# lowmee/xchu_slam

Hardware: AMD Instinct MI355X
Metric: NDT scans/sec (120k-pt scan vs 200k-voxel localmap, 30 iters) at 1/2/4/8 GPUs; % HBM BW (higher is better)
Workload: dtype f32 (f64 accumulate)

## Files before the change

### xchu_slam_amd/csrc/host_sort.hip

```cpp
#include "ndt_host.h"

namespace ndt::host {

ndt_status scan_ctx(ndt_ctx* c, Lane L, int nb, ScanCtx* sc) {
    sc->tickets = c->opt.tile_tickets ? 1 : 0;
    if ((size_t)nb > L.s.scan_status.cap) {
        TRY(ensure(c, L.s.scan_status, (size_t)nb));
        HIPCHK(c, hipMemsetAsync(L.s.scan_status.p, 0, L.s.scan_status.cap * sizeof(unsigned long long), L.st));
    }
    if (!L.s.scan_ticket.p) {
        TRY(ensure(c, L.s.scan_ticket, 1));
        HIPCHK(c, hipMemsetAsync(L.s.scan_ticket.p, 0, sizeof(unsigned long long), L.st));
        L.s.scan_tickets = 0;
    }
    sc->status = L.s.scan_status.p;
    sc->ticket = L.s.scan_ticket.p;
    sc->ticket_base = L.s.scan_tickets;
    sc->epoch = ++L.s.scan_epoch;
    sc->nb = nb;
    if (sc->tickets) L.s.scan_tickets += (unsigned long long)nb;
    return NDT_OK;
}

ndt_status enqueue_scan(ndt_ctx* c, Lane L, const int* in, int n_host, const int* n_dev, int* out, int* total_out, GridHeader* herr) {
    const int nb = std::max(1, ceil_div(n_host, kTileKeys));
    ScanCtx sc;
    TRY(scan_ctx(c, L, nb, &sc));
    hipLaunchKernelGGL(k_scan_onepass, dim3(nb), dim3(kBlock), 0, L.st, in, n_host, n_dev, out, total_out, sc, herr);
    return NDT_OK;
}

constexpr int kRadixWideKeys = 4 << 20;
int radix_items(const ndt_ctx* c, int n) {
    return ceil_div(n, kTileKeys) < c->n_cu ? 4 : (n >= kRadixWideKeys ? 24 : 16);
}
size_t radix_status_words(int nb) { return (size_t)4 * 256 * ((size_t)nb + (size_t)ceil_div(nb, 16)); }
void launch_radix_pass(const ndt_ctx* c, Lane L, int items, int nb, int* k0, int* v0, int* k1, int* v1, int n, int pass,
                       const GridHeader* h, GridHeader* herr, int last_pass) {
    auto* kern = items == 4 ? k_radix_onesweep<4> : items == 16 ? k_radix_onesweep<16> : k_radix_onesweep<24>;
    hipLaunchKernelGGL(kern, dim3(nb), dim3(kBlock), 0, L.st, k0, v0, k1, v1, n, pass, h, L.s.radix_aux.p, L.s.radix_status.p, nb,
                       herr, last_pass, c->opt.tile_tickets ? 1 : 0);
}

int radix_launch_passes(const ndt_ctx* c) {
    if (c->rerun_full) return 4;
    return c->opt.radix_force > 0 ? std::min(c->opt.radix_force, 4) : c->radix_pred;
}
void note_grid_width(ndt_ctx* c, long long cells, int dense) {
    if (cells <= 0) return;
    const long long top = dense ? cells - 1 : cells;
    int bits = 0;
    while (bits < 31 && (top >> bits) != 0) ++bits;
    c->radix_pred = std::min(4, std::max(1, (bits + 1 + 7) / 8));
}

ndt_status enqueue_bin_and_sort(ndt_ctx* c, Lane L, const float4* pts, int n, int dense, GridHeader* h, float leaf, int layout,
                                int binning, int2* cloud_span, int passes) {
    if (&L.s == &c->s && !cloud_span) c->inc_ok = false;
    const int nb_mm = std::max(1, std::min(ceil_div(n, 4 * kBlock), 1024));
    TRY(ensure(c, L.s.mm, (size_t)nb_mm * 7));
    const int items = radix_items(c, n);
    const int nb_sort = std::max(1, ceil_div(n, kBlock * items));
    const size_t n_kv = cloud_span ? (size_t)n + (size_t)n / 4 : (size_t)n;
    TRY(ensure(c, L.s.k0, n_kv)); TRY(ensure(c, L.s.v0, n_kv)); TRY(ensure(c, L.s.k1, n_kv)); TRY(ensure(c, L.s.v1, n_kv));
    TRY(ensure(c, L.s.radix_aux, kRadixAuxWords));
    TRY(ensure(c, L.s.radix_status, radix_status_words(nb_sort)));
    TRY(ensure(c, L.s.seg_start, (size_t)n + 1));
    hipLaunchKernelGGL(k_minmax, dim3(nb_mm), dim3(kBlock), 0, L.st, pts, n, dense, L.s.mm.p, L.s.radix_aux.p,
                       cloud_span ? c->d_clk.p + 3 : nullptr, nullptr, nullptr, nullptr);
    const int nb_keys = std::max(1, std::min(ceil_div(n, 4 * kBlock), 512));
    hipLaunchKernelGGL(k_keys, dim3(nb_keys), dim3(kBlock), 0, L.st, pts, n, dense, L.s.mm.p, nb_mm, h, leaf, c->prm.min_points_per_voxel,
                       c->prm.min_covar_eigvalue_mult, layout, binning, L.s.k0.p, L.s.v0.p, L.s.radix_aux.p, L.s.radix_status.p,
                       (int)radix_status_words(nb_sort), cloud_span ? c->grid.p : nullptr, (long long)c->grid.cap, cloud_span ? c->table.p : nullptr,
                       1LL << c->max_log2cap, nullptr, 0);
    for (int pass = 0; pass < passes; ++pass)
        launch_radix_pass(c, L, items, nb_sort, L.s.k0.p, L.s.v0.p, L.s.k1.p, L.s.v1.p, n, pass, h, h, passes - 1);
    const int nb_seg = std::max(1, ceil_div(n, kTileKeys));
    ScanCtx sc;
    TRY(scan_ctx(c, L, nb_seg, &sc));
    hipLaunchKernelGGL(k_seg_scan, dim3(nb_seg), dim3(kBlock), 0, L.st, L.s.k0.p, L.s.k1.p, n, h, L.s.seg_start.p, sc);
    if (cloud_span) {
        ScanCtx sc2;
        TRY(scan_ctx(c, L, nb_seg, &sc2));
        hipLaunchKernelGGL(k_cloud_scan, dim3(nb_seg), dim3(kBlock), 0, L.st, L.s.seg_start.p, n, h, cloud_span, sc2, c->max_log2cap);
    }
    return NDT_OK;
}

ndt_status enqueue_downsample_finalize(ndt_ctx* c, Lane L, const GridHeader* h, const float4* in, int n, float4* out) {
    TRY(ensure(c, L.s.sorted_pts, std::max(n, 1)));
    const int nb = std::max(1, std::min(ceil_div(n, 4 * kBlock), 2048));
    hipLaunchKernelGGL(k_sorted_gather, dim3(nb), dim3(kBlock), 0, L.st, in, L.s.v0.p, L.s.v1.p, h, L.s.sorted_pts.p, n);
    hipLaunchKernelGGL(k_downsample_finalize, dim3(std::max(1, ceil_div(n, kBlock))), dim3(kBlock), 0, L.st, L.s.sorted_pts.p,
                       L.s.seg_start.p, h, out);
    HIPCHK(c, hipGetLastError());
    return NDT_OK;
}

}
```

### xchu_slam_amd/csrc/host_target.hip

```cpp
#include "ndt_host.h"

namespace ndt::host {

namespace {

ndt_status grow_grid(ndt_ctx* c) {
    const long long want_cells = std::min<long long>(std::max<long long>(2 * c->grid_cells_seen, 16ll << 20), 1ll << 30);
    if ((long long)c->grid.cap < want_cells) TRY(ensure(c, c->grid, (size_t)want_cells));
    return NDT_OK;
}

ndt_status alloc_cloud_buffers(ndt_ctx* c, size_t max_cloud) {
    TRY(ensure(c, c->recs, max_cloud)); TRY(ensure(c, c->cent, max_cloud)); TRY(ensure(c, c->icovd, max_cloud * 9));
    TRY(ensure(c, c->evals, max_cloud * 3)); TRY(ensure(c, c->cloud_key, max_cloud));
    return NDT_OK;
}

constexpr int kFinalize3WavesMaxPoints = 4 << 20;

ndt_status prepare_target_buffers(ndt_ctx* c, int M, int* nb_cloud) {
    TRY(grow_grid(c));
    const size_t max_cloud = std::max(1, M / std::max(1, c->prm.min_points_per_voxel) + 1);
    TRY(alloc_cloud_buffers(c, max_cloud));
    unsigned l = 6;
    while (l < 30 && (1ull << l) < 4ull * max_cloud) ++l;
    c->max_log2cap = l;
    TRY(ensure(c, c->table, (size_t)1 << l));
    *nb_cloud = std::max(1, ceil_div((long long)max_cloud, kBlock));
    TRY(ensure(c, c->s.cloud_span, (size_t)*nb_cloud * kBlock));
    TRY(ensure(c, c->valid_part, max_cloud / 64 + 1));
    return NDT_OK;
}

ndt_status launch_finalize(ndt_ctx* c, int M, int nb_cloud) {
    auto* fin = M < kFinalize3WavesMaxPoints ? k_leaf_finalize<3> : k_leaf_finalize<2>;
    hipLaunchKernelGGL(fin, dim3(nb_cloud), dim3(kBlock), 0, c->stream.get(), c->target_ptr, c->s.k0.p, c->s.k1.p, c->s.v0.p,
                       c->s.v1.p, c->s.cloud_span.p, c->d_hdr.p, c->recs.p, c->cent.p, c->icovd.p, c->cloud_key.p,
                       c->evals.p, c->grid.p, c->table.p, c->valid_part.p);
    HIPCHK(c, hipGetLastError());
    return NDT_OK;
}

ndt_status enqueue_target_build(ndt_ctx* c) {
    c->inc_ok = false;
    ++c->n_builds_full;
    const int M = c->M;
    int nb_cloud = 0;
    TRY(prepare_target_buffers(c, M, &nb_cloud));
    TRY(enqueue_bin_and_sort(c, main_lane(c), c->target_ptr, M, c->target_dense, c->d_hdr.p, c->prm.resolution, 0, c->prm.precision_mode == 2 ? 1 : 0,
                             c->s.cloud_span.p, radix_launch_passes(c)));
    TRY(launch_finalize(c, M, nb_cloud));
    c->inc_ok = c->prm.precision_mode != 2 && c->target_dense == 1 && M > 0;
    return NDT_OK;
}

ndt_status enqueue_target_append(ndt_ctx* c, int n_old, int n_new, const float4* new_src) {
    const int M = n_old + n_new;
    int nb_cloud = 0;
    TRY(prepare_target_buffers(c, M, &nb_cloud));
    Lane Q{c->stream.get(), c->s_inc};
    float4* copy_to = new_src ? const_cast<float4*>(c->target_ptr) + n_old : nullptr;
    const float4* pts_new = new_src ? new_src : c->target_ptr + n_old;
    const int nq = std::max(n_new, 1);
    const int nb_mm = std::max(1, std::min(ceil_div(nq, 4 * kBlock), 1024));
    TRY(ensure(c, Q.s.mm, (size_t)nb_mm * 7));
    const int items = radix_items(c, nq);
    const int nb_sort = std::max(1, ceil_div(nq, kBlock * items));
    TRY(ensure(c, Q.s.k0, nq)); TRY(ensure(c, Q.s.v0, nq)); TRY(ensure(c, Q.s.k1, nq)); TRY(ensure(c, Q.s.v1, nq));
    TRY(ensure(c, Q.s.radix_aux, kRadixAuxWords));
    TRY(ensure(c, Q.s.radix_status, radix_status_words(nb_sort)));
    TRY(ensure(c, c->s.seg_start, (size_t)M + 1));
    hipLaunchKernelGGL(k_minmax, dim3(nb_mm), dim3(kBlock), 0, c->stream.get(), pts_new, n_new, 1, Q.s.mm.p, Q.s.radix_aux.p, c->d_clk.p + 3,
                       c->d_hdr.p, c->d_hdr_prev.p, copy_to);
    if (c->tgt_ev_valid) HIPCHK(c, hipEventRecord(c->ev_tgt.get(), c->stream.get()));
    const long long clear_words = std::max<long long>((long long)c->grid.cap, 2LL << c->max_log2cap) / 4;
    const int nb_keys = std::max(1, (int)std::min<long long>(std::max<long long>(ceil_div(nq, 4 * kBlock), ceil_div(clear_words, 4LL * kBlock)), 512));
    hipLaunchKernelGGL(k_keys, dim3(nb_keys), dim3(kBlock), 0, c->stream.get(), pts_new, n_new, 1, Q.s.mm.p, nb_mm, c->d_hdr.p, c->prm.resolution,
                       c->prm.min_points_per_voxel, c->prm.min_covar_eigvalue_mult, 0, 0, Q.s.k0.p, Q.s.v0.p, Q.s.radix_aux.p,
                       Q.s.radix_status.p, (int)radix_status_words(nb_sort), c->grid.p, (long long)c->grid.cap, c->table.p, 1LL << c->max_log2cap,
                       c->d_hdr_prev.p, n_old);
    const int passes = radix_launch_passes(c);
    for (int pass = 0; pass < passes; ++pass)
        launch_radix_pass(c, Q, items, nb_sort, Q.s.k0.p, Q.s.v0.p, Q.s.k1.p, Q.s.v1.p, n_new, pass, c->d_hdr.p, c->d_hdr.p, passes - 1);
    hipLaunchKernelGGL(k_merge_append, dim3(std::max(1, ceil_div(M, kMergeTileKeys))), dim3(kBlock), 0, c->stream.get(), c->s.k0.p, c->s.v0.p,
                       c->s.k1.p, c->s.v1.p, c->d_hdr_prev.p, n_old, Q.s.k0.p, Q.s.v0.p, Q.s.k1.p, Q.s.v1.p, n_new, c->d_hdr.p,
                       c->target_ptr);
    const Lane L = main_lane(c);
    const int nb_seg = std::max(1, ceil_div(M, kTileKeys));
    ScanCtx sc, sc2;
    TRY(scan_ctx(c, L, nb_seg, &sc));
    hipLaunchKernelGGL(k_seg_scan, dim3(nb_seg), dim3(kBlock), 0, c->stream.get(), c->s.k0.p, c->s.k1.p, M, c->d_hdr.p, c->s.seg_start.p, sc);
    TRY(scan_ctx(c, L, nb_seg, &sc2));
    hipLaunchKernelGGL(k_cloud_scan, dim3(nb_seg), dim3(kBlock), 0, c->stream.get(), c->s.seg_start.p, M, c->d_hdr.p, c->s.cloud_span.p, sc2,
                       c->max_log2cap);
    TRY(launch_finalize(c, M, nb_cloud));
    return NDT_OK;
}

}

ndt_status build_target(ndt_ctx* c) {
    ++c->tgt_gen;
    c->tgt_ev_valid = c->lanes.fit_tgt_used;
    if (c->tgt_ev_valid) HIPCHK(c, hipEventRecord(c->ev_tgt.get(), c->stream.get()));
    TRY(enqueue_target_build(c));
    c->build_unchecked = true;
    c->built_since_align = true;
    c->grid_valid = true;
    c->fit_valid = false;
    c->grid_res = c->prm.resolution;
    c->have_result = false;
    return NDT_OK;
}

ndt_status rerun_build(ndt_ctx* c, int berr) {
    ++c->n_builds_rerun;
    if (berr & kBuildErrLookback) {
        c->opt.tile_tickets = true;
        ++c->n_rerun_lookback;
    }
    c->inc_ok = false;
    c->rerun_full = true;
    const ndt_status st = build_target(c);
    c->rerun_full = false;
    return st;
}

ndt_status settle_build(ndt_ctx* c) {
    if (!c->build_unchecked || !c->grid_valid) return NDT_OK;
    for (int attempt = 0;; ++attempt) {
        HIPCHK(c, hipMemcpyAsync(c->h_hdr.get(), c->d_hdr.p, sizeof(GridHeader), hipMemcpyDeviceToHost, c->stream.get()));
        HIPCHK(c, hipStreamSynchronize(c->stream.get()));
        const int berr = c->h_hdr->pad[0];
        if (!berr) break;
        if (attempt > 0) return fail(c, NDT_EDEVICE, "target build failed twice (error bits " + std::to_string(berr) + ")");
        TRY(rerun_build(c, berr));
    }
    c->build_unchecked = false;
    note_grid_width(c, c->h_hdr->cells, c->target_dense);
    return NDT_OK;
}

ndt_status upload_points(ndt_ctx* c, DevBuf<float4>& dst, const float* xyz, size_t n, size_t stride_bytes) {
    TRY(ensure(c, dst, n));
    std::vector<float4> tmp(n);
    const char* base = reinterpret_cast<const char*>(xyz);
    for (size_t i = 0; i < n; ++i) {
        const float* f = reinterpret_cast<const float*>(base + i * stride_bytes);
        tmp[i] = make_float4(f[0], f[1], f[2], 1.0f);
    }
    if (n) HIPCHK(c, hipMemcpyAsync(dst.p, tmp.data(), n * sizeof(float4), hipMemcpyHostToDevice, c->stream.get()));
    HIPCHK(c, hipStreamSynchronize(c->stream.get()));
    return NDT_OK;
}

static ndt_status append_target(ndt_ctx* c, const float4* d_new, const float* h_new, size_t n, size_t stride_bytes) {
    TRY(set_dev(c));
    TRY(main_after_fit(c, false));
    if (n == 0) return NDT_OK;
    const size_t m0 = c->has_target ? (size_t)c->M : 0, m = m0 + n;
    if (m > 0x7fffffffULL) return fail(c, NDT_EINVAL, "target too large");
// ... 151 lines not shown
```

### xchu_slam_amd/csrc/ndt_kernels.h

```cpp
#pragma once
#include <hip/hip_runtime.h>
#include "ndt_types.h"
#include "ndt_linalg.h"
#include "ndt_icp.h"
#include "ndt_sc.h"
#include "ndt_isc.h"
#include "ndt_pgo.h"
#include "ndt_map.h"

namespace ndt {
__global__ void k_minmax(const float4*, int, int, float*, int*, unsigned long long*, const GridHeader*, GridHeader*, float4*);
__global__ void k_keys(const float4*, int, int, const float*, int, GridHeader*, float, int, double, int, int, int*, int*, int*, unsigned*, int,
                       int*, long long, int2*, long long, const GridHeader*, int);
__global__ void k_merge_append(int*, int*, int*, int*, const GridHeader*, int, const int*, const int*, const int*, const int*, int,
                               GridHeader*, const float4*);
template <int ITEMS>
__global__ void k_radix_onesweep(int*, int*, int*, int*, int, int, const GridHeader*, int*, unsigned*, int, GridHeader*, int, int);
__global__ void k_scan_onepass(const int*, int, const int*, int*, int*, ScanCtx, GridHeader*);
__global__ void k_seg_scan(const int*, const int*, int, GridHeader*, int*, ScanCtx);
__global__ void k_cloud_scan(const int*, int, GridHeader*, int2*, ScanCtx, unsigned);

template <int WAVES>
__global__ void k_leaf_finalize(const float4*, const int*, const int*, const int*, const int*, const int2*, GridHeader*,
                                VoxelRec*, float4*, double*, int*, double*, int*, int2*, int*);
__global__ void k_sorted_gather(const float4*, const int*, const int*, const GridHeader*, float4*, int);
__global__ void k_src_keys(const float4*, int, Mat4f, const GridHeader*, int*, int*, int*, unsigned*, int);
__global__ void k_src_gather(const float4*, const int*, const int*, const GridHeader*, float4*, int);
__global__ void k_crop_flags(const float4*, int, double, double, int*);
__global__ void k_compact4(const float4*, const int*, const int*, int, float4*);
template <int C>
__global__ void k_sor_knn(const float4*, int, int, const GridHeader*, const int*, const int*, const float4*, float*);
__global__ void k_sor_stats(const float*, int, double, double*);
__global__ void k_sor_keep(const float*, int, const double*, int*);
__global__ void k_ror_keep(const float4*, int, double, int, const GridHeader*, const int*, const int*, const float4*, int*);
__global__ void k_downsample_finalize(const float4*, const int*, const GridHeader*, float4*);
__global__ void k_fit_gather(const float4*, const int*, const int*, const int*, const int*, const int*, int, const GridHeader*, float4*,
                             int*, int*, int*);
__global__ void k_icp_pass(float4*, int, IcpState*, const GridHeader*, const int*, const int*, const float4*, const int*, int*, float*,
                           double*, unsigned*, IcpRecordDev*);
__global__ void k_sc_make(const float4*, int, unsigned*);
__global__ void k_sc_finalize(const unsigned*, ScDb, int);
__global__ void k_sc_detect(ScDb, const int*, const int*, int, int, ScDetectArgs, ndt_sc_result*);
__global__ void k_isc_make(const float4*, int, IscGeom, unsigned*);
__global__ void k_isc_finalize(const unsigned*, IscDb, int, int, int, double, double, double, double);
__global__ void k_isc_detect(IscDb, const int*, int, IscDetectArgs, IscPartial*);
__global__ void k_isc_reduce(const IscPartial*, const int*, int, int, IscDetectArgs, ndt_isc_result*);
__global__ void k_pgo_optimize(PgoGraph, PgoArgs);
__global__ void k_map_stack(const float4*, const int*, const long long*, const Mat4f*, int, int, int, float4*);
__global__ void k_fit_block_flags(const int*, const GridHeader*, int*);
__global__ void k_append2(const float4*, const float4*, int, const GridHeader*, float4*, float4*);
__global__ void k_fit_block_clear(int*, const GridHeader*);
__global__ void k_fit_tables(const int*, const int*, const int*, const int*, const GridHeader*, int*, int*);
__global__ void k_fitness(const float4*, int, Mat4f, const GridHeader*, const int*, const int*, const float4*, double, float*, double*,
                          int*, unsigned*, double*, long long*);
__global__ void k_score_radius(const float4*, int, Mat4f, const GridHeader*, const int2*, const int*, const VoxelRec*, const float4*,
                               const double*, double, double, double, float, double*);
template <int SEARCH, int PPT, bool ONE_TILE>
__global__ void k_pass_direct(const float4*, int, int, const GridHeader*, const int2*, const int*, const VoxelRec*, const AlignState*,
                              AlignState*, double*, unsigned*, double*, PassRecordDev*, int, int, unsigned long long*, int4*);
__global__ void k_pass_radius(const float4*, int, const GridHeader*, const int2*, const int*, const VoxelRec*, const float4*,
                              const double*, const AlignState*, AlignState*, double*, unsigned*, double*, PassRecordDev*, int, int,
                              unsigned long long*);
__global__ void k_transform(const float4*, int, const AlignState*, float4*);
__global__ void k_transform_mat(const float4*, int, Mat4f, float4*);
__global__ void k_align_init(const AlignState, AlignState*, unsigned*, unsigned long long*, int, unsigned long long*, const GridHeader*,
                             unsigned long long, const uint4*, uint4*, long long);
__global__ void k_copy16(const uint4*, uint4*, size_t);
__global__ void k_readback(const unsigned long long*, unsigned long long*, int, const unsigned long long*, unsigned long long*, int,
                           const unsigned long long*, unsigned long long*, int, const unsigned long long*, unsigned long long*,
                           unsigned long long*, unsigned long long, unsigned long long*, const GridHeader*);
hipError_t dbg_read_blk(unsigned long long* host, size_t count);
__global__ void k_svd_resume(AlignState*);
template <int SEARCH, bool ONE_TILE>
__global__ void k_pass_lead(const float4*, int, int, const GridHeader*, const int2*, const int*, const VoxelRec*, const AlignState*,
                            AlignState*, const double*, double*, PassRecordDev*, int, unsigned long long*, int4*);
}
```

### xchu_slam_amd/csrc/ndt_types.h

```cpp
#pragma once
#include <stdint.h>

namespace ndt {

constexpr int kBlock = 256;
constexpr int kLeadBlock = 512;
constexpr int kLeadBlock1 = 768;
#ifndef NDT_SPLIT_ACC
#define NDT_SPLIT_ACC 1
#endif
#ifndef NDT_LEAD_ONE_TILE
#define NDT_LEAD_ONE_TILE NDT_SPLIT_ACC
#endif
#ifndef NDT_DIRECT_ONE_TILE
#define NDT_DIRECT_ONE_TILE 0
#endif
constexpr int kDirectBlock = 256;
#ifndef NDT_PACKED_PAIR
#define NDT_PACKED_PAIR 1
#endif
#ifndef NDT_ROW_TRIPLE
#define NDT_ROW_TRIPLE 1
#endif
#ifndef NDT_NBR_CACHE
#define NDT_NBR_CACHE 1
#endif
__host__ __device__ constexpr int pass_block(int search, bool lead, bool one_tile = false) {
    return search == 1  ? kBlock : (lead ? (one_tile ? kLeadBlock1 : kLeadBlock) : kDirectBlock);
}
#ifndef NDT_PASS_WAVES
#define NDT_PASS_WAVES 2
#endif
__host__ __device__ constexpr int pass_waves(int search, int ppt, bool one_tile = false) {
    return search == 1 ? 1 : (ppt == 2 ? 2 : (one_tile ? 3 : NDT_PASS_WAVES));
}
__host__ __device__ constexpr int pass_wgs_per_cu(int search, bool lead, int ppt, bool one_tile = false) {
    return (search == 1 || lead) ? 1 : pass_waves(search, ppt, one_tile);
}
constexpr int kNumAcc = 44;
constexpr int kEmptyKey = -1;
constexpr int kRejectBit = 0x40000000;
__host__ __device__ constexpr int partial_stride(int nb) { return (nb + 1) & ~1; }
constexpr int kMaxHistory = 4096;
constexpr int kMaxGroups = 64;
constexpr int kGroupTicketStride = 32;
constexpr int kGroupTicketBase = 16;
constexpr int kPassCounterWords = kGroupTicketBase + kMaxGroups * kGroupTicketStride;
constexpr int kTwoLevelMinBlocks = 1024;
__host__ __device__ constexpr int group_size(int nb) {
    return nb / kMaxGroups >= 64 ? (((nb + kMaxGroups - 1) / kMaxGroups + 1) & ~1) : 64;
}
constexpr int kTsStride = 16;
constexpr int kRadixCopies = 8;
constexpr int kRadixAuxWords = kRadixCopies * 4 * 256 + 4;

enum PassKind { PASS_FULL = 0, PASS_GRAD = 1, PASS_HESS = 2 };
enum SearchMode { S_KDTREE = 0, S_DIRECT26 = 1, S_DIRECT7 = 2, S_DIRECT1 = 3 };

struct Mat4f {
    float m[16];
};

struct GridHeader {
    int min_b[4], max_b[4], div_b[4], divb_mul[4];
    float leaf[4], inv_leaf[4];
    float minp[4], maxp[4];
    int n_points;
    int n_leaves;
    int n_cloud;
    int n_valid;
    int overflow;
    int empty;
    int key_bits;
    int sentinel;
    unsigned log2cap;
    int min_points;
    double min_eig_mult;
    long long cells;
    int dense;
    int pad[2];
    int binning;
    int layout;
    int n_blocks_occ;
    int nblk[4];
    int flip;
    int pad2;
};
constexpr int kBuildErrLookback = 1;
constexpr int kBuildErrPasses = 2;
constexpr int kBuildErrMerge = 4;
constexpr int kMergeTileKeys = 2048;
constexpr int kFitBlockCells = 512;
#ifndef NDT_FIT_BLOCK
#define NDT_FIT_BLOCK 64
#endif
#ifndef NDT_FIT_TEAM
#define NDT_FIT_TEAM 16
#endif
static_assert(NDT_FIT_BLOCK >= 64, "k_fitness: a group's partials are reduced one per thread");
constexpr int kFitGroup = 64;
constexpr int kFitTicketStride = 64;
constexpr long long kFitMaxKeys = 1LL << 25;
constexpr int kFitMaxBlocks = (int)(kFitMaxKeys / kFitBlockCells);

struct __attribute__((aligned(16))) VoxelRec {
    double mean[3];
    float icov[9];
    int npts;
};
static_assert(sizeof(VoxelRec) == 64, "VoxelRec must be 64 B");

struct ScanCtx {
    unsigned long long* status;
    unsigned long long* ticket;
    unsigned long long ticket_base;
    unsigned epoch;
    int nb;
    int tickets;
};

struct PassRecordDev {
    int kind, newton_iter;
    double x[6];
    double score;
    double g[6];
    double H[36];
    long long pairs;
};

struct AlignState {
    double gauss_d1, gauss_d2, gauss_d3;
    double step_max, step_min, trans_eps;
    int max_iter, n_src, search, precision;
    int mt_possible;
    float radius;
    double p[6];
    double score, g[6], H[36];
    int nr_iterations, converged, done, phase;
    double dir[6], x_t[6];
    double phi_0, d_phi_0;
    double a_l, f_l, g_l, a_u, f_u, g_u, a_t;
    double phi_t, d_phi_t, psi_t, d_psi_t;
    int open_interval, interval_converged, step_iterations;
    int want_solve;
    int pending, pass_kind, solver_fallbacks, needs_tables;
    int needs_svd, svd_ready;
    int partials_pending;
    int build_error;
    double svd_dp[6];
    float T[16];
    float jang[8][4];
    float hang[16][4];
    double jang_d[8][3];
    double hang_d[15][3];
    double x_eval[6];
    double trans_probability;
    int n_passes, hist_count;
    long long pairs_total;
    long long grid_cells;
};

}
```

### xchu_slam_amd/csrc/voxel_build.hip

```cpp
#include "ndt_device.h"
#include "ndt_kernels.h"

namespace ndt {

constexpr int kTileItems = 16;
constexpr int kTile = kBlock * kTileItems;
constexpr int kRadixAux = kRadixAuxWords;

__global__ __launch_bounds__(kBlock) void k_minmax(const float4* __restrict__ pts, int n, int is_dense, float* __restrict__ part,
                                                   int* __restrict__ radix_aux, unsigned long long* __restrict__ clk_start,
                                                   const GridHeader* __restrict__ hdr_cur, GridHeader* __restrict__ hdr_save,
                                                   float4* __restrict__ copy_to) {
    if (clk_start && blockIdx.x == 0 && threadIdx.x == 0) *clk_start = __builtin_amdgcn_s_memrealtime();
    if (blockIdx.x == 0) {
        for (int i = threadIdx.x; i < kRadixAux; i += kBlock) radix_aux[i] = 0;
        if (hdr_save) {
            static_assert(sizeof(GridHeader) % 4 == 0 && sizeof(GridHeader) / 4 <= kBlock, "header copy: one word per thread");
            if (threadIdx.x < sizeof(GridHeader) / 4)
                reinterpret_cast<int*>(hdr_save)[threadIdx.x] = reinterpret_cast<const int*>(hdr_cur)[threadIdx.x];
        }
    }
    float mn[3] = {FLT_MAX, FLT_MAX, FLT_MAX}, mx[3] = {-FLT_MAX, -FLT_MAX, -FLT_MAX};
    int cnt = 0;
    const int stride = gridDim.x * kBlock;
    for (int i0 = blockIdx.x * kBlock + threadIdx.x; i0 < n; i0 += 4 * stride) {
        float4 q[4];
#pragma unroll
        for (int u = 0; u < 4; ++u) q[u] = i0 + u * stride < n ? pts[i0 + u * stride] : make_float4(0.f, 0.f, 0.f, 0.f);
        if (copy_to) {
#pragma unroll
            for (int u = 0; u < 4; ++u)
                if (i0 + u * stride < n) copy_to[i0 + u * stride] = q[u];
        }
#pragma unroll
        for (int u = 0; u < 4; ++u) {
            const float4 p = q[u];
            if (i0 + u * stride >= n) break;
            if (!is_dense && !(isfinite(p.x) && isfinite(p.y) && isfinite(p.z))) continue;
            mn[0] = fminf(mn[0], p.x); mn[1] = fminf(mn[1], p.y); mn[2] = fminf(mn[2], p.z);
            mx[0] = fmaxf(mx[0], p.x); mx[1] = fmaxf(mx[1], p.y); mx[2] = fmaxf(mx[2], p.z);
            ++cnt;
        }
    }
    __shared__ float s[kBlock][7];
    s[threadIdx.x][0] = mn[0]; s[threadIdx.x][1] = mn[1]; s[threadIdx.x][2] = mn[2];
    s[threadIdx.x][3] = mx[0]; s[threadIdx.x][4] = mx[1]; s[threadIdx.x][5] = mx[2];
    s[threadIdx.x][6] = __int_as_float(cnt);
    __syncthreads();
    for (int off = kBlock / 2; off > 0; off >>= 1) {
        if ((int)threadIdx.x < off) {
            const int o = threadIdx.x + off;
            for (int a = 0; a < 3; ++a) s[threadIdx.x][a] = fminf(s[threadIdx.x][a], s[o][a]);
            for (int a = 3; a < 6; ++a) s[threadIdx.x][a] = fmaxf(s[threadIdx.x][a], s[o][a]);
            s[threadIdx.x][6] = __int_as_float(__float_as_int(s[threadIdx.x][6]) + __float_as_int(s[o][6]));
        }
        __syncthreads();
    }
    if (threadIdx.x < 7) part[blockIdx.x * 7 + threadIdx.x] = s[0][threadIdx.x];
}

__device__ __forceinline__ void header_body(const float* __restrict__ part, int nb, GridHeader* h, float leaf, int min_pts, double eig_mult,
                                            int is_dense, int layout, int binning, float (*s)[7],
                                            const GridHeader* __restrict__ fold = nullptr) {
    float mn[3] = {FLT_MAX, FLT_MAX, FLT_MAX}, mx[3] = {-FLT_MAX, -FLT_MAX, -FLT_MAX};
    int cnt = 0;
    if (fold && threadIdx.x == 0) {
        for (int a = 0; a < 3; ++a) { mn[a] = fold->minp[a]; mx[a] = fold->maxp[a]; }
        cnt = fold->n_points;
    }
    for (int b = threadIdx.x; b < nb; b += kBlock) {
        for (int a = 0; a < 3; ++a) { mn[a] = fminf(mn[a], part[b * 7 + a]); mx[a] = fmaxf(mx[a], part[b * 7 + 3 + a]); }
        cnt += __float_as_int(part[b * 7 + 6]);
    }
    for (int a = 0; a < 3; ++a) { s[threadIdx.x][a] = mn[a]; s[threadIdx.x][3 + a] = mx[a]; }
    s[threadIdx.x][6] = __int_as_float(cnt);
    __syncthreads();
    for (int off = kBlock / 2; off > 0; off >>= 1) {
        if ((int)threadIdx.x < off) {
            const int o = threadIdx.x + off;
            for (int a = 0; a < 3; ++a) s[threadIdx.x][a] = fminf(s[threadIdx.x][a], s[o][a]);
            for (int a = 3; a < 6; ++a) s[threadIdx.x][a] = fmaxf(s[threadIdx.x][a], s[o][a]);
            s[threadIdx.x][6] = __int_as_float(__float_as_int(s[threadIdx.x][6]) + __float_as_int(s[o][6]));
        }
        __syncthreads();
    }
    if (threadIdx.x != 0) return;
    for (int a = 0; a < 3; ++a) { mn[a] = s[0][a]; mx[a] = s[0][3 + a]; }
    cnt = __float_as_int(s[0][6]);
    GridHeader g;
    for (int a = 0; a < 4; ++a) { g.min_b[a] = g.max_b[a] = g.div_b[a] = g.divb_mul[a] = 0; }
    for (int a = 0; a < 3; ++a) { g.leaf[a] = leaf; g.inv_leaf[a] = 1.0f / leaf; g.minp[a] = mn[a]; g.maxp[a] = mx[a]; }
    g.leaf[3] = 1.f; g.inv_leaf[3] = 1.f; g.minp[3] = g.maxp[3] = 0.f;
    g.n_points = cnt;
    g.n_leaves = g.n_cloud = g.n_valid = 0;
    g.overflow = 0;
    g.empty = 0;
    g.key_bits = 0;
    g.sentinel = 0;
    g.log2cap = 6;
    g.min_points = min_pts;
    g.min_eig_mult = eig_mult;
    g.cells = 0;
    g.dense = 0;
    g.pad[0] = g.pad[1] = 0;
    g.binning = binning;
    g.layout = layout;
    g.n_blocks_occ = 0;
    g.nblk[0] = g.nblk[1] = g.nblk[2] = g.nblk[3] = 0;
    g.flip = 0;
    g.pad2 = 0;
    if (cnt == 0) {
        g.empty = 1;
    } else if (layout == 1) {
        float cell = leaf;
        long long R = 0;
        for (int it = 0; it < 64; ++it) {
            const float inv = 1.0f / cell;
            long long nbk[3];
            for (int a = 0; a < 3; ++a) {
                g.min_b[a] = (int)floorf(mn[a] * inv);
                g.max_b[a] = (int)floorf(mx[a] * inv);
                g.div_b[a] = g.max_b[a] - g.min_b[a] + 1;
                nbk[a] = ((long long)g.div_b[a] + 7) >> 3;
            }
            R = nbk[0] * nbk[1] * nbk[2] * kFitBlockCells;
            if (R <= kFitMaxKeys && g.div_b[0] > 0 && g.div_b[1] > 0 && g.div_b[2] > 0) {
                for (int a = 0; a < 3; ++a) g.nblk[a] = (int)nbk[a];
                break;
            }
            cell *= 2.0f;
        }
        for (int a = 0; a < 3; ++a) { g.leaf[a] = cell; g.inv_leaf[a] = 1.0f / cell; }
        g.divb_mul[0] = 1;
        g.divb_mul[1] = g.div_b[0];
        g.divb_mul[2] = g.div_b[0] * g.div_b[1];
        g.cells = R;
        int bits = 0;
        const long long top = is_dense ? (R - 1) : R;
        while (bits < 31 && (top >> bits) != 0) ++bits;
        g.key_bits = bits;
        g.sentinel = is_dense ? 0x7fffffff : (int)((1LL << bits) - 1);
    } else {
        const long long dx = (long long)((mx[0] - mn[0]) * g.inv_leaf[0]) + 1;
        const long long dy = (long long)((mx[1] - mn[1]) * g.inv_leaf[1]) + 1;
        const long long dz = (long long)((mx[2] - mn[2]) * g.inv_leaf[2]) + 1;
        if (dx * dy * dz > 2147483647LL) {
            g.overflow = 1;
            g.empty = 1;
        } else {
            for (int a = 0; a < 3; ++a) {
                g.min_b[a] = binning ? (int)floorf(mn[a] / leaf) : (int)floorf(mn[a] * g.inv_leaf[a]);
                g.max_b[a] = binning ? (int)floorf(mx[a] / leaf) : (int)floorf(mx[a] * g.inv_leaf[a]);
                g.div_b[a] = g.max_b[a] - g.min_b[a] + 1;
            }
            g.divb_mul[0] = 1;
            g.divb_mul[1] = g.div_b[0];
            g.divb_mul[2] = g.div_b[0] * g.div_b[1];
            const long long D = (long long)g.div_b[0] * g.div_b[1] * g.div_b[2];
            g.cells = D;
            if (D > 2147483646LL) {
                g.overflow = 1;
                g.empty = 1;
            } else {
                int bits = 0;
                long long top = is_dense ? (D - 1) : D;
                while (bits < 31 && (top >> bits) != 0) ++bits;
                g.key_bits = bits;
                g.sentinel = is_dense ? 0x7fffffff : (int)((1LL << bits) - 1);
            }
        }
    }
    *h = g;
}

__device__ __forceinline__ int voxel_key(const float4 p, int is_dense, const GridHeader* __restrict__ h) {
    if (!is_dense && !(isfinite(p.x) && isfinite(p.y) && isfinite(p.z))) return h->sentinel;
    int ijk0, ijk1, ijk2;
    if (h->binning) {
        ijk0 = (int)floorf(p.x / h->leaf[0]) - h->min_b[0];
        ijk1 = (int)floorf(p.y / h->leaf[1]) - h->min_b[1];
        ijk2 = (int)floorf(p.z / h->leaf[2]) - h->min_b[2];
    } else {
        ijk0 = (int)(floorf(p.x * h->inv_leaf[0]) - (float)h->min_b[0]);
        ijk1 = (int)(floorf(p.y * h->inv_leaf[1]) - (float)h->min_b[1]);
        ijk2 = (int)(floorf(p.z * h->inv_leaf[2]) - (float)h->min_b[2]);
    }
    if (h->layout == 1)
        return ((((ijk2 >> 3) * h->nblk[1] + (ijk1 >> 3)) * h->nblk[0] + (ijk0 >> 3)) << 9) | ((ijk2 & 7) << 6) | ((ijk1 & 7) << 3) |
               (ijk0 & 7);
    return ijk0 * h->divb_mul[0] + ijk1 * h->divb_mul[1] + ijk2 * h->divb_mul[2];
}

__global__ __launch_bounds__(kBlock) void k_keys(const float4* __restrict__ pts, int n, int is_dense, const float* __restrict__ part, int nb_mm,
                                                 GridHeader* __restrict__ hout, float leaf, int min_pts, double eig_mult, int layout,
                                                 int binning, int* __restrict__ keys, int* __restrict__ vals,
                                                 int* __restrict__ radix_aux, unsigned* __restrict__ status, int status_words,
                                                 int* __restrict__ grid, long long grid_cap, int2* __restrict__ table, long long table_slots,
                                                 const GridHeader* __restrict__ fold, int val_base) {
    for (int i = blockIdx.x * kBlock + threadIdx.x; i < status_words; i += gridDim.x * kBlock) status[i] = 0u;
    __shared__ GridHeader s_h;
    __shared__ float s_red[kBlock][7];
    header_body(part, nb_mm, &s_h, leaf, min_pts, eig_mult, is_dense, layout, binning, s_red, fold);
    __syncthreads();
    const bool lookup = grid != nullptr && !s_h.empty;
    const bool dense = lookup && s_h.cells > 0 && s_h.cells <= grid_cap;
    if (blockIdx.x == 0 && threadIdx.x == 0) {
        GridHeader g = s_h;
        g.dense = dense ? 1 : 0;
        *hout = g;
    }
    const GridHeader* h = &s_h;
    if (h->empty) return;
    if (lookup) {
        const long long words = dense ? s_h.cells : 2 * table_slots;
        const int4 fill = dense ? make_int4(-1, -1, -1, -1) : make_int4(kEmptyKey, 0, kEmptyKey, 0);
        int4* dst = dense ? reinterpret_cast<int4*>(grid) : reinterpret_cast<int4*>(table);
        const long long m4 = words / 4;
        for (long long i = (long long)blockIdx.x * kBlock + threadIdx.x; i < m4; i += (long long)gridDim.x * kBlock) dst[i] = fill;
        if (blockIdx.x == 0 && threadIdx.x < (int)(words - 4 * m4)) {
            int* w = dense ? grid : reinterpret_cast<int*>(table);
            w[4 * m4 + threadIdx.x] = (threadIdx.x & 1) && !dense ? 0 : -1;
        }
    }
    const int passes = (h->key_bits + 7) / 8;
    __shared__ int cnt[4][256];
    for (int q = 0; q < 4; ++q) cnt[q][threadIdx.x] = 0;
    __syncthreads();
    const int stride = gridDim.x * kBlock;
    for (int i0 = blockIdx.x * kBlock + threadIdx.x; i0 < n; i0 += 4 * stride) {
        float4 p[4];
#pragma unroll
        for (int u = 0; u < 4; ++u) p[u] = i0 + u * stride < n ? pts[i0 + u * stride] : make_float4(0.f, 0.f, 0.f, 0.f);
#pragma unroll
        for (int u = 0; u < 4; ++u) {
            const int i = i0 + u * stride;
            if (i >= n) break;
            const int key = voxel_key(p[u], is_dense, h);
            keys[i] = key;
            vals[i] = val_base + i;
            for (int q = 0; q < passes; ++q) atomicAdd(&cnt[q][(key >> (8 * q)) & 255], 1);
        }
    }
    __syncthreads();
    for (int q = 0; q < passes; ++q) {
        const int c = cnt[q][threadIdx.x];
        if (c) atomicAdd(&radix_aux[(blockIdx.x % kRadixCopies) * 1024 + q * 256 + threadIdx.x], c);
    }
}

__device__ __forceinline__ bool radix_pass_active(const GridHeader* h, int pass) { return !h->empty && 8 * pass < h->key_bits; }

constexpr unsigned kStAgg = 1u << 30;
constexpr unsigned kStPre = 2u << 30;
constexpr unsigned kStCnt = (1u << 30) - 1u;
constexpr int kSpinLimit = 1 << 15;
#ifndef NDT_TWOLEVEL_TILES
#define NDT_TWOLEVEL_TILES 1024
#endif
constexpr int kTwoLevelTiles = NDT_TWOLEVEL_TILES, kGroupTiles = 16;

#ifdef NDT_SORT_STAMPS
constexpr int kSortStampWords = 16;
__device__ unsigned long long g_sort_ts[3 * 4 * 3 * kSortStampWords];
#define NDT_SORT_STAMP_BEGIN()                                                                                              \
    const int sort_cls = tile == 0 ? 0 : tile == nb - 1 ? 2 : tile == nb / 2 ? 1 : -1;                                      \
    unsigned long long* sort_row =                                                                                          \
        tid == 0 && sort_cls >= 0 ? &g_sort_ts[(((ITEMS == 4 ? 0 : ITEMS == 16 ? 1 : 2) * 4 + pass) * 3 + sort_cls) * kSortStampWords] \
                                  : nullptr;                                                                                \
    const unsigned long long sort_t0 = __builtin_amdgcn_s_memrealtime();                                                    \
    if (sort_row) { sort_row[0] += 1ull; sort_row[6] = (unsigned long long)nb; sort_row[8] = sort_t0; }
#define NDT_SORT_STAMP(slot)                                                  \
    do {                                                                      \
        __syncthreads();                                                      \
        if (sort_row) {                                                       \
            const unsigned long long _n = __builtin_amdgcn_s_memrealtime();   \
            sort_row[(slot)] += _n - sort_t0;                                 \
            sort_row[8 + (slot)] = _n;                                        \
        }                                                                     \
    } while (0)
#else
#define NDT_SORT_STAMP_BEGIN() do { } while (0)
#define NDT_SORT_STAMP(slot) do { } while (0)
#endif

template <int N>
__device__ __forceinline__ void status_load(unsigned (&wd)[N], const unsigned* base, int stride, int cnt, int tid) {
    asm volatile("" : "+s"(base));
#pragma unroll
    for (int u = 0; u < N; ++u)
        wd[u] = u < cnt ? __hip_atomic_load(base + (ptrdiff_t)u * stride + tid, __ATOMIC_RELAXED, __HIP_MEMORY_SCOPE_AGENT) : kStAgg;
}
template <int N>
__device__ __forceinline__ bool status_take(const unsigned (&wd)[N], unsigned* sum) {
    bool all = true;
    unsigned s = 0;
#pragma unroll
    for (int u = 0; u < N; ++u) {
        all = all && (wd[u] & ~kStCnt) != 0u;
        s += wd[u] & kStCnt;
    }
    if (all) *sum += s;
    return all;
}

template <int ITEMS>
__global__ __launch_bounds__(kBlock) void k_radix_onesweep(int* __restrict__ k0, int* __restrict__ v0, int* __restrict__ k1,
                                                           int* __restrict__ v1, int n, int pass, const GridHeader* h,
                                                           int* __restrict__ radix_aux, unsigned* __restrict__ status, int nb,
                                                           GridHeader* __restrict__ herr, int last_pass, int tickets) {
    static_assert(kBlock == 256, "thread = digit");
    if (pass == last_pass && pass < 3 && blockIdx.x == 0 && threadIdx.x == 0 && radix_pass_active(h, pass + 1))
        atomicOr(&herr->pad[0], kBuildErrPasses);
    if (!radix_pass_active(h, pass)) return;
    const int* kin = (pass & 1) ? k1 : k0;
    const int* vin = (pass & 1) ? v1 : v0;
    int* kout = (pass & 1) ? k0 : k1;
    int* vout = (pass & 1) ? v0 : v1;
    constexpr int NW = kBlock / 64;
    constexpr int TILE = ITEMS * kBlock;
    constexpr bool kStage = ITEMS >= 16;
    const int tid = threadIdx.x, lane = tid & 63, w = tid >> 6;
    const int shift = 8 * pass;
    __shared__ int s_tile;
    __shared__ int wcnt[NW][256];
// ... 1044 lines not shown
```

Before: 1306.

## Prefetch point loads and use wavefront-shuffle reductions in minmax/keys front end

Restructures the minmax and key-generation kernels so each thread issues a batch of clamped point loads up front and double-buffers the next batch while processing the current one. In k_keys, the partial-header row loads and the first point batch are hoisted ahead of the header reduction, which overlaps that latency. The shared-memory tree reductions are replaced with xor-shuffle wavefront reductions, and the grid sizes are changed (minmax capped at 256 workgroups, keys at 1024). In exchange it uses more registers per thread, reads clamped duplicate addresses at the tail, and k_keys assumes the partial count fits in a fixed rows-per-thread bound.

```diff
diff --git a/xchu_slam_amd/csrc/host_sort.hip b/xchu_slam_amd/csrc/host_sort.hip
--- a/xchu_slam_amd/csrc/host_sort.hip
+++ b/xchu_slam_amd/csrc/host_sort.hip
@@ -57,7 +57,7 @@
 ndt_status enqueue_bin_and_sort(ndt_ctx* c, Lane L, const float4* pts, int n, int dense, GridHeader* h, float leaf, int layout,
                                 int binning, int2* cloud_span, int passes) {
     if (&L.s == &c->s && !cloud_span) c->inc_ok = false;
-    const int nb_mm = std::max(1, std::min(ceil_div(n, 4 * kBlock), 1024));
+    const int nb_mm = front_wgs(n, kMinmaxMaxWgs);
     TRY(ensure(c, L.s.mm, (size_t)nb_mm * 7));
     const int items = radix_items(c, n);
     const int nb_sort = std::max(1, ceil_div(n, kBlock * items));
@@ -66,13 +66,12 @@
     TRY(ensure(c, L.s.radix_aux, kRadixAuxWords));
     TRY(ensure(c, L.s.radix_status, radix_status_words(nb_sort)));
     TRY(ensure(c, L.s.seg_start, (size_t)n + 1));
+    const HeaderSpec spec{leaf, c->prm.min_points_per_voxel, c->prm.min_covar_eigvalue_mult, layout, binning};
     hipLaunchKernelGGL(k_minmax, dim3(nb_mm), dim3(kBlock), 0, L.st, pts, n, dense, L.s.mm.p, L.s.radix_aux.p,
                        cloud_span ? c->d_clk.p + 3 : nullptr, nullptr, nullptr, nullptr);
-    const int nb_keys = std::max(1, std::min(ceil_div(n, 4 * kBlock), 512));
-    hipLaunchKernelGGL(k_keys, dim3(nb_keys), dim3(kBlock), 0, L.st, pts, n, dense, L.s.mm.p, nb_mm, h, leaf, c->prm.min_points_per_voxel,
-                       c->prm.min_covar_eigvalue_mult, layout, binning, L.s.k0.p, L.s.v0.p, L.s.radix_aux.p, L.s.radix_status.p,
-                       (int)radix_status_words(nb_sort), cloud_span ? c->grid.p : nullptr, (long long)c->grid.cap, cloud_span ? c->table.p : nullptr,
-                       1LL << c->max_log2cap, nullptr, 0);
+    hipLaunchKernelGGL(k_keys, dim3(front_wgs(n, kKeysMaxWgs)), dim3(kBlock), 0, L.st, pts, n, dense, L.s.mm.p, nb_mm, h, spec, L.s.k0.p, L.s.v0.p,
+                       L.s.radix_aux.p, L.s.radix_status.p, (int)radix_status_words(nb_sort), cloud_span ? c->grid.p : nullptr,
+                       (long long)c->grid.cap, cloud_span ? c->table.p : nullptr, 1LL << c->max_log2cap, nullptr, 0);
     for (int pass = 0; pass < passes; ++pass)
         launch_radix_pass(c, L, items, nb_sort, L.s.k0.p, L.s.v0.p, L.s.k1.p, L.s.v1.p, n, pass, h, h, passes - 1);
     const int nb_seg = std::max(1, ceil_div(n, kTileKeys));
diff --git a/xchu_slam_amd/csrc/host_target.hip b/xchu_slam_amd/csrc/host_target.hip
--- a/xchu_slam_amd/csrc/host_target.hip
+++ b/xchu_slam_amd/csrc/host_target.hip
@@ -62,7 +62,7 @@
     float4* copy_to = new_src ? const_cast<float4*>(c->target_ptr) + n_old : nullptr;
     const float4* pts_new = new_src ? new_src : c->target_ptr + n_old;
     const int nq = std::max(n_new, 1);
-    const int nb_mm = std::max(1, std::min(ceil_div(nq, 4 * kBlock), 1024));
+    const int nb_mm = front_wgs(nq, kMinmaxMaxWgs);
     TRY(ensure(c, Q.s.mm, (size_t)nb_mm * 7));
     const int items = radix_items(c, nq);
     const int nb_sort = std::max(1, ceil_div(nq, kBlock * items));
@@ -70,13 +70,13 @@
     TRY(ensure(c, Q.s.radix_aux, kRadixAuxWords));
     TRY(ensure(c, Q.s.radix_status, radix_status_words(nb_sort)));
     TRY(ensure(c, c->s.seg_start, (size_t)M + 1));
+    const HeaderSpec spec{(float)c->prm.resolution, c->prm.min_points_per_voxel, c->prm.min_covar_eigvalue_mult, 0, 0};
     hipLaunchKernelGGL(k_minmax, dim3(nb_mm), dim3(kBlock), 0, c->stream.get(), pts_new, n_new, 1, Q.s.mm.p, Q.s.radix_aux.p, c->d_clk.p + 3,
                        c->d_hdr.p, c->d_hdr_prev.p, copy_to);
     if (c->tgt_ev_valid) HIPCHK(c, hipEventRecord(c->ev_tgt.get(), c->stream.get()));
     const long long clear_words = std::max<long long>((long long)c->grid.cap, 2LL << c->max_log2cap) / 4;
-    const int nb_keys = std::max(1, (int)std::min<long long>(std::max<long long>(ceil_div(nq, 4 * kBlock), ceil_div(clear_words, 4LL * kBlock)), 512));
-    hipLaunchKernelGGL(k_keys, dim3(nb_keys), dim3(kBlock), 0, c->stream.get(), pts_new, n_new, 1, Q.s.mm.p, nb_mm, c->d_hdr.p, c->prm.resolution,
-                       c->prm.min_points_per_voxel, c->prm.min_covar_eigvalue_mult, 0, 0, Q.s.k0.p, Q.s.v0.p, Q.s.radix_aux.p,
+    const int nb_keys = std::max(1, (int)std::min<long long>(std::max<long long>(ceil_div(nq, 4 * kBlock), ceil_div(clear_words, 4LL * kBlock)), kKeysMaxWgs));
+    hipLaunchKernelGGL(k_keys, dim3(nb_keys), dim3(kBlock), 0, c->stream.get(), pts_new, n_new, 1, Q.s.mm.p, nb_mm, c->d_hdr.p, spec, Q.s.k0.p, Q.s.v0.p, Q.s.radix_aux.p,
                        Q.s.radix_status.p, (int)radix_status_words(nb_sort), c->grid.p, (long long)c->grid.cap, c->table.p, 1LL << c->max_log2cap,
                        c->d_hdr_prev.p, n_old);
     const int passes = radix_launch_passes(c);
diff --git a/xchu_slam_amd/csrc/ndt_kernels.h b/xchu_slam_amd/csrc/ndt_kernels.h
--- a/xchu_slam_amd/csrc/ndt_kernels.h
+++ b/xchu_slam_amd/csrc/ndt_kernels.h
@@ -10,8 +10,8 @@
 
 namespace ndt {
 __global__ void k_minmax(const float4*, int, int, float*, int*, unsigned long long*, const GridHeader*, GridHeader*, float4*);
-__global__ void k_keys(const float4*, int, int, const float*, int, GridHeader*, float, int, double, int, int, int*, int*, int*, unsigned*, int,
-                       int*, long long, int2*, long long, const GridHeader*, int);
+__global__ void k_keys(const float4*, int, int, const float*, int, GridHeader*, HeaderSpec, int*, int*, int*, unsigned*, int, int*, long long,
+                       int2*, long long, const GridHeader*, int);
 __global__ void k_merge_append(int*, int*, int*, int*, const GridHeader*, int, const int*, const int*, const int*, const int*, int,
                                GridHeader*, const float4*);
 template <int ITEMS>
diff --git a/xchu_slam_amd/csrc/ndt_types.h b/xchu_slam_amd/csrc/ndt_types.h
--- a/xchu_slam_amd/csrc/ndt_types.h
+++ b/xchu_slam_amd/csrc/ndt_types.h
@@ -86,6 +86,25 @@
     int flip;
     int pad2;
 };
+#ifndef NDT_FRONT_LOADS
+#define NDT_FRONT_LOADS 8
+#endif
+#ifndef NDT_MM_WGS
+#define NDT_MM_WGS 256
+#endif
+#ifndef NDT_KEYS_WGS
+#define NDT_KEYS_WGS 1024
+#endif
+constexpr int kFrontLoads = NDT_FRONT_LOADS;
+constexpr int kMinmaxMaxWgs = NDT_MM_WGS;
+constexpr int kKeysMaxWgs = NDT_KEYS_WGS;
+struct HeaderSpec {
+    float leaf;
+    int min_pts;
+    double eig_mult;
+    int layout, binning;
+};
+constexpr int front_wgs(int n, int cap) { return n <= 4 * kBlock ? 1 : ((n - 1) / (4 * kBlock) + 1 < cap ? (n - 1) / (4 * kBlock) + 1 : cap); }
 constexpr int kBuildErrLookback = 1;
 constexpr int kBuildErrPasses = 2;
 constexpr int kBuildErrMerge = 4;
diff --git a/xchu_slam_amd/csrc/voxel_build.hip b/xchu_slam_amd/csrc/voxel_build.hip
--- a/xchu_slam_amd/csrc/voxel_build.hip
+++ b/xchu_slam_amd/csrc/voxel_build.hip
@@ -7,6 +7,74 @@
 constexpr int kTile = kBlock * kTileItems;
 constexpr int kRadixAux = kRadixAuxWords;
 
+struct Box {
+    float mn[3], mx[3];
+    int cnt;
+};
+__device__ __forceinline__ Box box_none() { return Box{{FLT_MAX, FLT_MAX, FLT_MAX}, {-FLT_MAX, -FLT_MAX, -FLT_MAX}, 0}; }
+__device__ __forceinline__ void box_join(Box& b, const Box& o) {
+#pragma unroll
+    for (int a = 0; a < 3; ++a) { b.mn[a] = fminf(b.mn[a], o.mn[a]); b.mx[a] = fmaxf(b.mx[a], o.mx[a]); }
+    b.cnt += o.cnt;
+}
+__device__ __forceinline__ Box box_block_reduce(Box b, float (*s)[7]) {
+#pragma unroll
+    for (int m = 32; m > 0; m >>= 1) {
+        Box o;
+#pragma unroll
+        for (int a = 0; a < 3; ++a) { o.mn[a] = __shfl_xor(b.mn[a], m); o.mx[a] = __shfl_xor(b.mx[a], m); }
+        o.cnt = __shfl_xor(b.cnt, m);
+        box_join(b, o);
+    }
+    const int w = threadIdx.x >> 6;
+    if ((threadIdx.x & 63) == 0) {
+#pragma unroll
+        for (int a = 0; a < 3; ++a) { s[w][a] = b.mn[a]; s[w][3 + a] = b.mx[a]; }
+        s[w][6] = __int_as_float(b.cnt);
+    }
+    __syncthreads();
+    Box r = box_none();
+#pragma unroll
+    for (int q = 0; q < kBlock / 64; ++q) {
+        Box o;
+#pragma unroll
+        for (int a = 0; a < 3; ++a) { o.mn[a] = s[q][a]; o.mx[a] = s[q][3 + a]; }
+        o.cnt = __float_as_int(s[q][6]);
+        box_join(r, o);
+    }
+    return r;
+}
+
+__device__ __forceinline__ void front_load(float4 (&q)[kFrontLoads], const float4* __restrict__ pts, int i0, int stride, int n) {
+#pragma unroll
+    for (int u = 0; u < kFrontLoads; ++u) q[u] = pts[min(i0 + u * stride, n - 1)];
+}
+
+__device__ __forceinline__ GridHeader make_header(const Box& box, const HeaderSpec& spec, int is_dense);
+constexpr int kRowsPerThread = (kMinmaxMaxWgs + kBlock - 1) / kBlock;
+__device__ __forceinline__ void rows_load(const float* __restrict__ part, int nb, float (&v)[kRowsPerThread][7]) {
+#pragma unroll
+    for (int r = 0; r < kRowsPerThread; ++r) {
+        const int b = threadIdx.x + r * kBlock;
+#pragma unroll
+        for (int a = 0; a < 7; ++a) {
+            v[r][a] = part[min(b, nb - 1) * 7 + a];
+        }
+        v[r][6] = __int_as_float(__float_as_int(v[r][6]) & -(int)(b < nb));
+    }
+}
+__device__ __forceinline__ Box rows_box(const float (&v)[kRowsPerThread][7], const GridHeader* __restrict__ fold, float (*s)[7]) {
+    static_assert(sizeof(GridHeader) % 4 == 0 && sizeof(GridHeader) / 4 <= kBlock, "header copies: one word per thread");
+    Box t = box_none();
+    if (fold && threadIdx.x == 0) {
+        for (int a = 0; a < 3; ++a) { t.mn[a] = fold->minp[a]; t.mx[a] = fold->maxp[a]; }
+        t.cnt = fold->n_points;
+    }
+#pragma unroll
+    for (int r = 0; r < kRowsPerThread; ++r)
+        box_join(t, Box{{v[r][0], v[r][1], v[r][2]}, {v[r][3], v[r][4], v[r][5]}, __float_as_int(v[r][6])});
+    return box_block_reduce(t, s);
+}
 __global__ __launch_bounds__(kBlock) void k_minmax(const float4* __restrict__ pts, int n, int is_dense, float* __restrict__ part,
                                                    int* __restrict__ radix_aux, unsigned long long* __restrict__ clk_start,
                                                    const GridHeader* __restrict__ hdr_cur, GridHeader* __restrict__ hdr_save,
@@ -15,78 +83,53 @@
     if (blockIdx.x == 0) {
         for (int i = threadIdx.x; i < kRadixAux; i += kBlock) radix_aux[i] = 0;
         if (hdr_save) {
-            static_assert(sizeof(GridHeader) % 4 == 0 && sizeof(GridHeader) / 4 <= kBlock, "header copy: one word per thread");
             if (threadIdx.x < sizeof(GridHeader) / 4)
                 reinterpret_cast<int*>(hdr_save)[threadIdx.x] = reinterpret_cast<const int*>(hdr_cur)[threadIdx.x];
         }
     }
-    float mn[3] = {FLT_MAX, FLT_MAX, FLT_MAX}, mx[3] = {-FLT_MAX, -FLT_MAX, -FLT_MAX};
-    int cnt = 0;
+    Box box = box_none();
     const int stride = gridDim.x * kBlock;
-    for (int i0 = blockIdx.x * kBlock + threadIdx.x; i0 < n; i0 += 4 * stride) {
-        float4 q[4];
-#pragma unroll
-        for (int u = 0; u < 4; ++u) q[u] = i0 + u * stride < n ? pts[i0 + u * stride] : make_float4(0.f, 0.f, 0.f, 0.f);
+    const float4* src = n > 0 ? pts : reinterpret_cast<const float4*>(part);
+    const int n1 = max(n, 1);
+    int i0 = blockIdx.x * kBlock + threadIdx.x;
+    float4 q[kFrontLoads];
+    front_load(q, src, i0, stride, n1);
+    while (i0 < n) {
+        const int i1 = i0 + kFrontLoads * stride;
+        float4 nx[kFrontLoads];
+        front_load(nx, src, i1, stride, n1);
         if (copy_to) {
 #pragma unroll
-            for (int u = 0; u < 4; ++u)
+            for (int u = 0; u < kFrontLoads; ++u)
                 if (i0 + u * stride < n) copy_to[i0 + u * stride] = q[u];
         }
 #pragma unroll
-        for (int u = 0; u < 4; ++u) {
+        for (int u = 0; u < kFrontLoads; ++u) {
             const float4 p = q[u];
-            if (i0 + u * stride >= n) break;
-            if (!is_dense && !(isfinite(p.x) && isfinite(p.y) && isfinite(p.z))) continue;
-            mn[0] = fminf(mn[0], p.x); mn[1] = fminf(mn[1], p.y); mn[2] = fminf(mn[2], p.z);
-            mx[0] = fmaxf(mx[0], p.x); mx[1] = fmaxf(mx[1], p.y); mx[2] = fmaxf(mx[2], p.z);
-            ++cnt;
-        }
-    }
-    __shared__ float s[kBlock][7];
-    s[threadIdx.x][0] = mn[0]; s[threadIdx.x][1] = mn[1]; s[threadIdx.x][2] = mn[2];
-    s[threadIdx.x][3] = mx[0]; s[threadIdx.x][4] = mx[1]; s[threadIdx.x][5] = mx[2];
-    s[threadIdx.x][6] = __int_as_float(cnt);
-    __syncthreads();
-    for (int off = kBlock / 2; off > 0; off >>= 1) {
-        if ((int)threadIdx.x < off) {
-            const int o = threadIdx.x + off;
-            for (int a = 0; a < 3; ++a) s[threadIdx.x][a] = fminf(s[threadIdx.x][a], s[o][a]);
-            for (int a = 3; a < 6; ++a) s[threadIdx.x][a] = fmaxf(s[threadIdx.x][a], s[o][a]);
-            s[threadIdx.x][6] = __int_as_float(__float_as_int(s[threadIdx.x][6]) + __float_as_int(s[o][6]));
-        }
-        __syncthreads();
-    }
-    if (threadIdx.x < 7) part[blockIdx.x * 7 + threadIdx.x] = s[0][threadIdx.x];
-}
-
-__device__ __forceinline__ void header_body(const float* __restrict__ part, int nb, GridHeader* h, float leaf, int min_pts, double eig_mult,
-                                            int is_dense, int layout, int binning, float (*s)[7],
-                                            const GridHeader* __restrict__ fold = nullptr) {
-    float mn[3] = {FLT_MAX, FLT_MAX, FLT_MAX}, mx[3] = {-FLT_MAX, -FLT_MAX, -FLT_MAX};
-    int cnt = 0;
-    if (fold && threadIdx.x == 0) {
-        for (int a = 0; a < 3; ++a) { mn[a] = fold->minp[a]; mx[a] = fold->maxp[a]; }
-        cnt = fold->n_points;
-    }
-    for (int b = threadIdx.x; b < nb; b += kBlock) {
-        for (int a = 0; a < 3; ++a) { mn[a] = fminf(mn[a], part[b * 7 + a]); mx[a] = fmaxf(mx[a], part[b * 7 + 3 + a]); }
-        cnt += __float_as_int(part[b * 7 + 6]);
-    }
-    for (int a = 0; a < 3; ++a) { s[threadIdx.x][a] = mn[a]; s[threadIdx.x][3 + a] = mx[a]; }
-    s[threadIdx.x][6] = __int_as_float(cnt);
-    __syncthreads();
-    for (int off = kBlock / 2; off > 0; off >>= 1) {
-        if ((int)threadIdx.x < off) {
-            const int o = threadIdx.x + off;
-            for (int a = 0; a < 3; ++a) s[threadIdx.x][a] = fminf(s[threadIdx.x][a], s[o][a]);
-            for (int a = 3; a < 6; ++a) s[threadIdx.x][a] = fmaxf(s[threadIdx.x][a], s[o][a]);
-            s[threadIdx.x][6] = __int_as_float(__float_as_int(s[threadIdx.x][6]) + __float_as_int(s[o][6]));
-        }
-        __syncthreads();
-    }
-    if (threadIdx.x != 0) return;
-    for (int a = 0; a < 3; ++a) { mn[a] = s[0][a]; mx[a] = s[0][3 + a]; }
-    cnt = __float_as_int(s[0][6]);
+            const bool take = i0 + u * stride < n && (is_dense || (isfinite(p.x) && isfinite(p.y) && isfinite(p.z)));
+            box_join(box, Box{{take ? p.x : FLT_MAX, take ? p.y : FLT_MAX, take ? p.z : FLT_MAX},
+                              {take ? p.x : -FLT_MAX, take ? p.y : -FLT_MAX, take ? p.z : -FLT_MAX}, take ? 1 : 0});
+        }
+#pragma unroll
+        for (int u = 0; u < kFrontLoads; ++u) q[u] = nx[u];
+        i0 = i1;
+    }
+    __shared__ float s[kBlock / 64][7];
+    box = box_block_reduce(box, s);
+    if (threadIdx.x < 7) {
+        const int t = threadIdx.x;
+        const float v = t == 0 ? box.mn[0] : t == 1 ? box.mn[1] : t == 2 ? box.mn[2] : t == 3 ? box.mx[0] : t == 4 ? box.mx[1] : t == 5 ? box.mx[2]
+                                                                                                                               : __int_as_float(box.cnt);
+        part[blockIdx.x * 7 + t] = v;
+    }
+}
+
+__device__ __forceinline__ GridHeader make_header(const Box& box, const HeaderSpec& spec, int is_dense) {
+    const float leaf = spec.leaf;
+    const int layout = spec.layout, binning = spec.binning;
+    const float* mn = box.mn;
+    const float* mx = box.mx;
+    const int cnt = box.cnt;
     GridHeader g;
     for (int a = 0; a < 4; ++a) { g.min_b[a] = g.max_b[a] = g.div_b[a] = g.divb_mul[a] = 0; }
     for (int a = 0; a < 3; ++a) { g.leaf[a] = leaf; g.inv_leaf[a] = 1.0f / leaf; g.minp[a] = mn[a]; g.maxp[a] = mx[a]; }
@@ -98,8 +141,8 @@
     g.key_bits = 0;
     g.sentinel = 0;
     g.log2cap = 6;
-    g.min_points = min_pts;
-    g.min_eig_mult = eig_mult;
+    g.min_points = spec.min_pts;
+    g.min_eig_mult = spec.eig_mult;
     g.cells = 0;
     g.dense = 0;
     g.pad[0] = g.pad[1] = 0;
@@ -170,7 +213,7 @@
             }
         }
     }
-    *h = g;
+    return g;
 }
 
 __device__ __forceinline__ int voxel_key(const float4 p, int is_dense, const GridHeader* __restrict__ h) {
@@ -191,16 +234,33 @@
     return ijk0 * h->divb_mul[0] + ijk1 * h->divb_mul[1] + ijk2 * h->divb_mul[2];
 }
 
+__device__ __forceinline__ void clear16(int4* __restrict__ dst, long long m4, const int4 fill) {
+    for (long long i = (long long)blockIdx.x * kBlock + threadIdx.x; i < m4; i += (long long)gridDim.x * kBlock) dst[i] = fill;
+}
 __global__ __launch_bounds__(kBlock) void k_keys(const float4* __restrict__ pts, int n, int is_dense, const float* __restrict__ part, int nb_mm,
-                                                 GridHeader* __restrict__ hout, float leaf, int min_pts, double eig_mult, int layout,
-                                                 int binning, int* __restrict__ keys, int* __restrict__ vals,
+                                                 GridHeader* __restrict__ hout, HeaderSpec spec, int* __restrict__ keys, int* __restrict__ vals,
                                                  int* __restrict__ radix_aux, unsigned* __restrict__ status, int status_words,
                                                  int* __restrict__ grid, long long grid_cap, int2* __restrict__ table, long long table_slots,
                                                  const GridHeader* __restrict__ fold, int val_base) {
-    for (int i = blockIdx.x * kBlock + threadIdx.x; i < status_words; i += gridDim.x * kBlock) status[i] = 0u;
     __shared__ GridHeader s_h;
-    __shared__ float s_red[kBlock][7];
-    header_body(part, nb_mm, &s_h, leaf, min_pts, eig_mult, is_dense, layout, binning, s_red, fold);
+    __shared__ int cnt[4][256];
+    const int stride = gridDim.x * kBlock;
+    int i0 = blockIdx.x * kBlock + threadIdx.x;
+    float4 p[kFrontLoads];
+    const float4* src = n > 0 ? pts : reinterpret_cast<const float4*>(part);
+    const int n1 = max(n, 1);
+    __shared__ float s_red[kBlock / 64][7];
+    float rows[kRowsPerThread][7];
+    rows_load(part, nb_mm, rows);
+    front_load(p, src, i0, stride, n1);
+    const Box all = rows_box(rows, fold, s_red);
+    if (threadIdx.x == 0) s_h = make_header(all, spec, is_dense);
+    for (int q = 0; q < 4; ++q) cnt[q][threadIdx.x] = 0;
+    {
+        const long long s4 = status_words / 4;
+        clear16(reinterpret_cast<int4*>(status), s4, make_int4(0, 0, 0, 0));
+        if (blockIdx.x == 0 && (int)threadIdx.x < status_words - 4 * (int)s4) status[4 * s4 + threadIdx.x] = 0u;
+    }
     __syncthreads();
     const bool lookup = grid != nullptr && !s_h.empty;
     const bool dense = lookup && s_h.cells > 0 && s_h.cells <= grid_cap;
@@ -211,28 +271,24 @@
     }
     const GridHeader* h = &s_h;
     if (h->empty) return;
+    const long long words = dense ? s_h.cells : 2 * table_slots;
+    const int4 fill = dense ? make_int4(-1, -1, -1, -1) : make_int4(kEmptyKey, 0, kEmptyKey, 0);
+    int4* dst = dense ? reinterpret_cast<int4*>(grid) : reinterpret_cast<int4*>(table);
+    const long long m4 = words / 4;
     if (lookup) {
-        const long long words = dense ? s_h.cells : 2 * table_slots;
-        const int4 fill = dense ? make_int4(-1, -1, -1, -1) : make_int4(kEmptyKey, 0, kEmptyKey, 0);
-        int4* dst = dense ? reinterpret_cast<int4*>(grid) : reinterpret_cast<int4*>(table);
-        const long long m4 = words / 4;
-        for (long long i = (long long)blockIdx.x * kBlock + threadIdx.x; i < m4; i += (long long)gridDim.x * kBlock) dst[i] = fill;
+        clear16(dst, m4, fill);
         if (blockIdx.x == 0 && threadIdx.x < (int)(words - 4 * m4)) {
             int* w = dense ? grid : reinterpret_cast<int*>(table);
             w[4 * m4 + threadIdx.x] = (threadIdx.x & 1) && !dense ? 0 : -1;
         }
     }
     const int passes = (h->key_bits + 7) / 8;
-    __shared__ int cnt[4][256];
-    for (int q = 0; q < 4; ++q) cnt[q][threadIdx.x] = 0;
-    __syncthreads();
-    const int stride = gridDim.x * kBlock;
-    for (int i0 = blockIdx.x * kBlock + threadIdx.x; i0 < n; i0 += 4 * stride) {
-        float4 p[4];
-#pragma unroll
-        for (int u = 0; u < 4; ++u) p[u] = i0 + u * stride < n ? pts[i0 + u * stride] : make_float4(0.f, 0.f, 0.f, 0.f);
-#pragma unroll
-        for (int u = 0; u < 4; ++u) {
+    while (i0 < n) {
+        const int i1 = i0 + kFrontLoads * stride;
+        float4 nx[kFrontLoads];
+        front_load(nx, src, i1, stride, n1);
+#pragma unroll
+        for (int u = 0; u < kFrontLoads; ++u) {
             const int i = i0 + u * stride;
             if (i >= n) break;
             const int key = voxel_key(p[u], is_dense, h);
@@ -240,6 +296,9 @@
             vals[i] = val_base + i;
             for (int q = 0; q < passes; ++q) atomicAdd(&cnt[q][(key >> (8 * q)) & 255], 1);
         }
+#pragma unroll
+        for (int u = 0; u < kFrontLoads; ++u) p[u] = nx[u];
+        i0 = i1;
     }
     __syncthreads();
     for (int q = 0; q < passes; ++q) {
```

Result: no change. 1312 (median of 6 runs) (+0.4%).
